# 2alaaa/distributed-llm-scheduler

Measured on AMD Instinct MI355X. Metric: DAG makespan (ms) + tasks completed under mem cap, GPT-2 DAG at 1/2/4/8 MI355X, lower is better.
Workload: dtype bf16

## Files before the change

csrc/kernels/gemm_glds_impl.h:

```cpp
#pragma once
#include <cstdlib>
#include <type_traits>
#include "common.h"
#include "kernels.h"
#include "gemm_glds_cfgs.h"

#ifndef DLS_STAMP
#define DLS_STAMP(k)
#endif

namespace {

__device__ __forceinline__ int kslice_count(int K, int kslice) { return K / kslice; }

template <int N>
__device__ __forceinline__ void wait_vm() {
  asm volatile("s_waitcnt vmcnt(%0)" ::"n"(N) : "memory");
}
template <int PW, int A>
__device__ __forceinline__ void wait_tiles(int ahead) {
  if constexpr (A == 0) {
    wait_vm<0>();
  } else {
    if (ahead >= A) wait_vm<PW * A>();
// ... 1347 lines not shown
using C31 = Cfg<192, 128, 2, 2, 2, 0, 1>;
using C32 = Cfg<192, 128, 2, 2, 3, 0, 1>;
using C33 = Cfg<192, 128, 4, 2, 3, 0, 1>;
using C34 = Cfg<256, 256, 2, 4, 2, 0, 0, 1, 1>;
using C35 = Cfg<256, 256, 2, 4, 2, 1, 0, 1, 1>;
using C36 = Cfg<256, 224, 4, 2, 2, 0, 1>;
using C37 = Cfg<256, 224, 8, 1, 2, 0, 1>;
using C38 = Cfg<128, 96, 4, 2, 4>;
using C39 = Cfg<128, 96, 2, 2, 2, 0, 0, 2>;
using C40 = Cfg<128, 64, 2, 2, 3, 0, 0, 2>;
using C41 = Cfg<192, 128, 4, 2, 3, 0, 2>;
using C42 = Cfg<256, 144, 8, 1, 3>;
using C43 = Cfg<256, 192, 4, 2, 2, 0, 1>;
using C44 = Cfg<160, 256, 2, 4, 2, 0, 1>;
using C45 = Cfg<32, 48, 2, 1, 3, 0, 0, 4>;
using C46 = Cfg<128, 128, 2, 2, 2, 0, 0, 1, 0, 2>;
using C47 = Cfg<128, 128, 2, 2, 2, 0, 1, 1, 0, 2>;

template <>
struct TallTile<C44> {
  using type = Cfg<224, 256, 2, 4, 2, 0, 1>;
};
template <>
struct TallTile<C33> {
  using type = C14;
};

template <class C>
void grouped(const GemmArgs& a, int n_groups, const int* offsets, const unsigned long long* w_ptrs,
             const unsigned long long* c_ptrs, hipStream_t s, const int* a_rows) {
  static const int w_stream = [] {
    const char* e = std::getenv("DLS_EXPERT_NT");
    return e && e[0] == '0' ? 0 : 1;
  }();
  const char* pe = std::getenv("DLS_EXPERT_PAIRS");
  const int pairs = pe && *pe ? std::atoi(pe) : 2;
  const int pair = a.grouped_shared ? 0 : pairs;
  const char* xe = std::getenv("DLS_EXPERT_XCD");
  const bool xcd = xe && *xe == '1' && !a.grouped_shared && pair != 1;
  const char* te = std::getenv("DLS_EXPERT_TALL");
  const bool tall = !(te && *te == '0') && !a.grouped_shared;
  const Epi ep{a.rope, nullptr, nullptr, nullptr, w_ptrs, c_ptrs,
               (a.grouped_shared ? 8 : ((size_t)a.M * a.lda * 2 < (1ull << 31) ? w_stream : 0)) |
                   (pair == 1 ? 16 : pair == 2 ? 32 : pair == 3 ? 64 : 0) | (xcd ? 128 : 0) | (tall ? 256 : 0)};
  const int tiles_n = (a.N + C::BN - 1) / C::BN;
  const int blocks = pair == 1 ? (n_groups * tiles_n + 7) / 8 * 16 : pair >= 2 ? 2 * n_groups * tiles_n
                                                                               : n_groups * tiles_n;
  hipLaunchKernelGGL((gemm_glds_kernel<C, 0, 3>), dim3(blocks), dim3(C::T), 0, s, (const bf16*)a.A, a.lda,
                     nullptr, a.ldw, (bf16*)a.C, a.ldc, nullptr, nullptr, 0,
                     const_cast<float*>(reinterpret_cast<const float*>(a_rows)), a.M, a.N, a.K, a.act, a.alpha,
                     n_groups, tiles_n, 1, a.K, nullptr, 0, 1e-5f, offsets, a.compact_rows, ep);
}

}

#define DLS_GLDS_DEFINE(ID)                                                                                     \
  bool glds_launch_cfg##ID(const GemmArgs& a, int splitk, float* ws, hipStream_t s, const float* ln_colsum,     \
                           int ln_mode, float ln_eps, const int* rows, bool persist) {                          \
    return launch<C##ID>(a, splitk, ws, s, ln_colsum, ln_mode, ln_eps, rows, persist);                          \
  }                                                                                                             \
  void glds_grouped_cfg##ID(const GemmArgs& a, int n_groups, const int* offsets, const unsigned long long* w_ptrs, \
                            const unsigned long long* c_ptrs, hipStream_t s, const int* a_rows) {               \
    grouped<C##ID>(a, n_groups, offsets, w_ptrs, c_ptrs, s, a_rows);                                            \
  }
```

csrc/kernels/kernels.h:

```cpp
#pragma once

#include <hip/hip_runtime_api.h>
#include <stdint.h>

constexpr int kActSwiglu = 4;

struct RopeArgs {
  const float* cos = nullptr;
  const float* sin = nullptr;
  int S = 1, D = 2, cols = 0;
};

struct GemmArgs {
  const void* A;
  int lda;
  const void* W;
  int ldw;
  void* C;
  int ldc;
  const void* bias;
  const void* R;
  int ldr;
  int M, N, K;
  int act;
  float alpha;
  int config;
  int compact_rows = 0;
  int grouped_shared = 0;
  RopeArgs rope{};
  float* stats_out = nullptr;
  const float* ext_stats = nullptr;
  int* tile_sem = nullptr;
  void* norm_out = nullptr;
  const void* norm_w = nullptr;
  const void* norm_b = nullptr;
  int norm_mode = 0;
  float norm_eps = 1e-5f;
  int ldn = 0;
  int stream_pol = 0;
};

struct Epi {
  RopeArgs rope;
  float* stats_out;
  const float* ext_stats;
  int* tile_sem = nullptr;
  const unsigned long long* grp_w = nullptr;
  const unsigned long long* grp_c = nullptr;
  int w_stream = 0;
};

int gemm_pick_config(int M, int N, int K);
void launch_gemm_bf16(const GemmArgs& a, hipStream_t s);

int gemm_glds_num_configs();
int gemm_glds_kstep(int cfg);
void gemm_glds_tile(int cfg, int* bm, int* bn);
int gemm_glds_resolve(int cfg, int act, bool ln_in);
constexpr int kGemmPersist = 64;
void gemm_glds_pick(int M, int N, int K, int* cfg, int* splitk);
size_t gemm_glds_workspace_bytes(int M, int N, int splitk);
bool launch_gemm_glds(const GemmArgs& a, int cfg, int splitk, void* workspace, hipStream_t s,
                      const float* ln_colsum = nullptr, int ln_mode = 0, float ln_eps = 1e-5f,
                      const int* rows = nullptr);
void launch_gemm_glds_grouped(const GemmArgs& a, int cfg, int n_groups, const int* offsets,
                              const unsigned long long* w_ptrs, const unsigned long long* c_ptrs, hipStream_t s,
                              const int* a_rows = nullptr);

struct GemmW8Args {
  const void* A;
  int lda;
  const void* Wq;
  int ldw;
  const float* scale;
  void* C;
  int ldc;
  const void* bias;
  const void* R;
  int ldr;
  int M, N, K;
  int act;
  float alpha;
  int config;
  int splitk;
  float* workspace;
  int store_pol;
};
int gemm_w8_num_configs();
void gemm_w8_pick(int M, int N, int K, int* cfg, int* splitk);
int gemm_w8_max_splitk(int cfg, int K);
size_t gemm_w8_workspace_bytes(int M, int N, int splitk);
void launch_gemm_w8(const GemmW8Args& a, hipStream_t s);

struct GemmW8GroupedArgs {
  const void* A;
  int lda;
  const int* a_rows;
  const int* offsets;
  const unsigned long long* w_ptrs;
  const unsigned long long* s_ptrs;
  const unsigned long long* c_ptrs;
  void* C;
  int ldc;
  int compact_rows;
  int R, N, K;
  int act;
  int n_groups;
  int config;
  int shared_weights;
  int store_pol;
};
int gemm_w8_grouped_num_configs();
int gemm_w8_grouped_tile_rows(int cfg);
int gemm_w8_grouped_pick(int rows_hint, int N, int K, int n_groups);
void launch_gemm_w8_grouped(const GemmW8GroupedArgs& a, hipStream_t s);

struct GemmW8A8Args {
// ... 269 lines not shown
```

csrc/kernels/ops_binding.cpp:

```cpp
#include <cstdlib>

#include <torch/extension.h>
#include <c10/hip/HIPStream.h>

#include "kernels.h"

namespace {

hipStream_t cur_stream() { return c10::hip::getCurrentHIPStream().stream(); }

constexpr int64_t kSemPool = 1 << 20;
int64_t sem_next[64];
int* split_k_counters(const at::Tensor& like, int64_t n) {
  static at::Tensor* pool = new at::Tensor[64];
  int64_t* next = sem_next;
  const int d = like.get_device();
  TORCH_CHECK(d >= 0 && d < 64 && n <= kSemPool, "split-K counters");
  if (!pool[d].defined()) pool[d] = at::zeros({kSemPool}, like.options().dtype(at::kInt));
  n = (n + 63) / 64 * 64;
  if (next[d] + n > kSemPool) next[d] = 0;
  int* p = pool[d].data_ptr<int>() + next[d];
  next[d] += n;
  return p;
}
int64_t split_k_cursor(int64_t device) {
  TORCH_CHECK(device >= 0 && device < 64, "split-K counters");
  return sem_next[device];
}
const bool kSplitKFixup = [] {
  const char* e = std::getenv("DLS_SPLITK_FIXUP");
  return !(e && e[0] == '0');
}();

void check_bf16(const at::Tensor& t, const char* name) {
  TORCH_CHECK(t.is_cuda(), name, " must be a GPU tensor");
  TORCH_CHECK(t.scalar_type() == at::kBFloat16, name, " must be bfloat16");
}

void check_rows(const at::Tensor& t, const char* name) {
  TORCH_CHECK(t.dim() == 2, name, " must be 2-D");
  TORCH_CHECK(t.stride(1) == 1, name, " must have contiguous rows");
  TORCH_CHECK(t.stride(0) % 8 == 0, name, " row stride must be a multiple of 8 elements");
  TORCH_CHECK(reinterpret_cast<uintptr_t>(t.data_ptr()) % 16 == 0, name, " must be 16-byte aligned");
}

at::Tensor as2d(const at::Tensor& t) { return t.dim() == 2 ? t : t.reshape({-1, t.size(-1)}); }

constexpr int64_t kRegStage = 100;

at::Tensor gemm(const at::Tensor& a_in, const at::Tensor& w, const c10::optional<at::Tensor>& bias,
                const c10::optional<at::Tensor>& residual, int64_t act, double alpha,
                const c10::optional<at::Tensor>& out, int64_t config, int64_t splitk,
                const c10::optional<at::Tensor>& ln_colsum, int64_t ln_mode, double ln_eps,
                const c10::optional<at::Tensor>& rows, bool compact_rows,
                const c10::optional<at::Tensor>& rope_cos, const c10::optional<at::Tensor>& rope_sin, int64_t rope_S,
                int64_t rope_D, int64_t rope_cols, const c10::optional<at::Tensor>& stats_out,
                const c10::optional<at::Tensor>& ext_stats, const c10::optional<at::Tensor>& norm_out,
                const c10::optional<at::Tensor>& norm_w, const c10::optional<at::Tensor>& norm_b, int64_t norm_mode,
                double norm_eps, int64_t stream_pol) {
  check_bf16(a_in, "A");
  check_bf16(w, "W");
  TORCH_CHECK(config < kRegStage + 4, "unknown GEMM config ", config, " (register-staged configs are ", kRegStage,
              "..", kRegStage + 3, ")");
  at::Tensor a = as2d(a_in);
  check_rows(a, "A");
  check_rows(w, "W");
  const int64_t M = a.size(0), K = a.size(1), N = w.size(0);
  const bool swiglu = act == kActSwiglu;
  const int64_t NO = swiglu ? N / 2 : N;
  TORCH_CHECK(w.size(1) == K, "W must be [N][K] with K = ", K, ", got ", w.sizes());
  TORCH_CHECK(K % 8 == 0, "K must be a multiple of 8");
  TORCH_CHECK(!swiglu || (N % 32 == 0 && K % 64 == 0 && !residual.has_value()),
              "SwiGLU epilogue needs N % 32 == 0, K % 64 == 0 and no residual");
  at::Tensor c;
  if (out.has_value()) {
    c = as2d(*out);
    check_bf16(c, "out");
    TORCH_CHECK((c.size(0) == M || (compact_rows && c.size(0) <= M)) && c.size(1) == NO && c.stride(1) == 1,
                "out must be [M][N_out] (or fewer rows with compact_rows)");
  } else {
    c = at::empty({M, NO}, a.options());
  }
  const void* bptr = nullptr;
  if (bias.has_value()) {
    check_bf16(*bias, "bias");
    TORCH_CHECK(bias->is_contiguous() && bias->numel() == N, "bias must be contiguous [N]");
    bptr = bias->data_ptr();
  }
  const void* rptr = nullptr;
  int ldr = 0;
  if (residual.has_value()) {
    at::Tensor r = as2d(*residual);
    check_bf16(r, "residual");
    TORCH_CHECK(r.size(0) == M && r.size(1) == N && r.stride(1) == 1, "residual must be [M][N]");
    rptr = r.data_ptr();
    ldr = (int)r.stride(0);
  }
  const int* rowp = nullptr;
  if (rows.has_value()) {
    TORCH_CHECK(rows->scalar_type() == at::kInt && rows->numel() == 2 && rows->is_contiguous() &&
                    rows->device() == a.device(),
                "rows must be a contiguous int32[2] device tensor");
    TORCH_CHECK(K % 64 == 0 && ln_mode == 0, "row-ranged GEMM needs K % 64 == 0 and no folded norm");
    rowp = rows->data_ptr<int>();
  }
  if (M == 0 || N == 0) return c;
  GemmArgs g{a.data_ptr(), (int)a.stride(0), w.data_ptr(), (int)w.stride(0), c.data_ptr(), (int)c.stride(0),
             bptr, rptr, ldr, (int)M, (int)N, (int)K, (int)act, (float)alpha, -1,
             (compact_rows && rows.has_value()) ? (int)c.size(0) : 0};
  g.stream_pol = (int)stream_pol;
  at::Tensor y_n;
  if (norm_out.has_value()) {
    TORCH_CHECK(norm_mode == 1 || norm_mode == 2, "norm_mode: 1 LayerNorm, 2 RMSNorm");
    TORCH_CHECK(!swiglu && !rows.has_value() && c.is_contiguous(), "post-norm needs a full, contiguous output");
    TORCH_CHECK(N % 8 == 0 && N <= 8192, "post-norm needs N % 8 == 0 and N <= 8192, got N = ", N);
    y_n = as2d(*norm_out);
    check_bf16(y_n, "norm_out");
    TORCH_CHECK(y_n.is_contiguous() && y_n.size(0) == M && y_n.size(1) == N, "norm_out must be contiguous [M][N]");
    TORCH_CHECK(norm_w.has_value() && norm_w->is_contiguous() && norm_w->numel() == N, "norm_w [N]");
    check_bf16(*norm_w, "norm_w");
    TORCH_CHECK(norm_mode == 2 || (norm_b.has_value() && norm_b->is_contiguous() && norm_b->numel() == N),
                "LayerNorm post-norm needs norm_b [N]");
    g.norm_out = y_n.data_ptr();
    g.ldn = (int)N;
    g.norm_w = norm_w->data_ptr();
    g.norm_b = norm_mode == 1 ? norm_b->data_ptr() : nullptr;
    g.norm_mode = (int)norm_mode;
    g.norm_eps = (float)norm_eps;
  }
  auto post_norm = [&](bool done) {
    if (!norm_out.has_value() || done) return;
    if (norm_mode == 2)
      launch_rmsnorm(c.data_ptr(), nullptr, nullptr, g.norm_w, y_n.data_ptr(), (int)M, (int)N, (float)norm_eps,
                     cur_stream());
    else
      launch_layernorm(c.data_ptr(), nullptr, nullptr, g.norm_w, g.norm_b, y_n.data_ptr(), (int)M, (int)N,
                       (float)norm_eps, cur_stream());
  };
  TORCH_CHECK(!compact_rows || (rows.has_value() && !residual.has_value()), "compact_rows needs rows and no residual");
  auto check_stats = [&](const at::Tensor& t, const char* name) {
    TORCH_CHECK(t.is_cuda() && t.scalar_type() == at::kFloat && t.is_contiguous() && t.numel() == 2 * M, name,
                " must be a contiguous fp32 [M][2] GPU tensor");
  };
  if (stats_out.has_value()) {
    check_stats(*stats_out, "stats_out");
    TORCH_CHECK(!swiglu && !rows.has_value(), "row statistics are emitted by plain (non-SwiGLU, full-row) GEMMs");
    g.stats_out = stats_out->data_ptr<float>();
  }
  if (ext_stats.has_value()) {
    check_stats(*ext_stats, "ext_stats");
    TORCH_CHECK(ln_mode != 0, "ext_stats needs ln_mode (1 LayerNorm, 2 RMSNorm) and ln_colsum");
    g.ext_stats = ext_stats->data_ptr<float>();
  }
  if (rope_cols > 0) {
    TORCH_CHECK(rope_cos.has_value() && rope_sin.has_value() && rope_cos->scalar_type() == at::kFloat &&
                    rope_sin->scalar_type() == at::kFloat && rope_cos->is_contiguous() && rope_sin->is_contiguous() &&
                    rope_cos->is_cuda() && rope_sin->is_cuda() &&
                    rope_cos->numel() >= rope_S * rope_D / 2 && rope_sin->numel() >= rope_S * rope_D / 2,
                "RoPE epilogue: cos/sin fp32 [S][D/2]");
    TORCH_CHECK(rope_D % 4 == 0 && rope_cols % rope_D == 0 && rope_cols <= N && !swiglu && K % 64 == 0 &&
                    !rows.has_value() && act == 0,
                "RoPE epilogue: D % 4 == 0, whole heads, LDS-DMA kernel, no activation / SwiGLU / row range");
    g.rope = RopeArgs{rope_cos->data_ptr<float>(), rope_sin->data_ptr<float>(), (int)rope_S, (int)rope_D,
                      (int)rope_cols};
    if (config >= kRegStage) config = -1;
  }
  const bool glds_ok = (K % 64 == 0);
  const float* csp = nullptr;
  if (ln_mode != 0) {
    TORCH_CHECK(glds_ok, "fused norm-GEMM needs K % 64 == 0");
    TORCH_CHECK(ln_colsum.has_value() && ln_colsum->scalar_type() == at::kFloat && ln_colsum->is_contiguous() &&
                    ln_colsum->numel() == N,
                "fused norm-GEMM needs fp32 ln_colsum [N]");
    csp = ln_colsum->data_ptr<float>();
  }
  if (ln_mode != 0 || swiglu || rowp || stats_out.has_value()) {
    TORCH_CHECK(glds_ok, "this epilogue needs the LDS-DMA kernel (K % 64 == 0)");
    if (config >= kRegStage) config = -1;
  }
  if (config >= kRegStage || !glds_ok) {
    g.config = config >= kRegStage ? (int)(config - kRegStage) : -1;
    launch_gemm_bf16(g, cur_stream());
    post_norm(false);
    return c;
  }
  int cfg = (int)config, sk = (int)splitk;
  if (cfg < 0 || sk <= 0) {
    int acfg, ask;
    gemm_glds_pick((int)M, (int)N, (int)K, &acfg, &ask);
    if (cfg < 0) cfg = acfg;
    if (sk <= 0) sk = ask;
  }
  TORCH_CHECK((cfg & (kGemmPersist - 1)) < gemm_glds_num_configs() && cfg < 2 * kGemmPersist, "unknown GEMM config ", cfg);
  TORCH_CHECK(K % gemm_glds_kstep(cfg) == 0, "GEMM config ", cfg, " needs K % ", gemm_glds_kstep(cfg), " == 0");
  const bool split_ok = (N % 8 == 0) && (c.stride(0) % 8 == 0) && (ldr % 8 == 0) &&
                        K % (gemm_glds_kstep(cfg) * sk) == 0 &&
                        (!swiglu || N % 32 == 0);
  if (!split_ok || (ln_mode != 0 && !ext_stats.has_value())) sk = 1;
  at::Tensor ws;
  if (sk > 1) {
    ws = at::empty({(int64_t)gemm_glds_workspace_bytes((int)M, (int)N, sk) / 4}, a.options().dtype(at::kFloat));
    if (kSplitKFixup && !rowp && !norm_out.has_value()) {
      int bm, bn;
      gemm_glds_tile(gemm_glds_resolve(cfg, (int)act, false), &bm, &bn);
      g.tile_sem = split_k_counters(a, (M + bm - 1) / bm * ((N + bn - 1) / bn));
    }
  }
  post_norm(launch_gemm_glds(g, cfg, sk, sk > 1 ? ws.data_ptr() : nullptr, cur_stream(), csp, (int)ln_mode,
                             (float)ln_eps, rowp));
  return c;
}

at::Tensor gemm_w8(const at::Tensor& a_in, const at::Tensor& wq, const at::Tensor& scale,
                   const c10::optional<at::Tensor>& bias, const c10::optional<at::Tensor>& residual, int64_t act,
                   double alpha, const c10::optional<at::Tensor>& out, int64_t config, int64_t splitk,
                   int64_t store_pol, const c10::optional<at::Tensor>& workspace) {
  check_bf16(a_in, "A");
  at::Tensor a = as2d(a_in);
  check_rows(a, "A");
  TORCH_CHECK(wq.is_cuda() && wq.device() == a.device() && wq.scalar_type() == at::kFloat8_e4m3fn,
              "W must be a float8_e4m3fn tensor on A's GPU");
  TORCH_CHECK(wq.dim() == 2, "W must be 2-D");
  const int64_t M = a.size(0), K = a.size(1), N = wq.size(0);
  TORCH_CHECK(wq.size(1) == K, "W must be [N][K] with K = ", K, ", got ", wq.sizes());
  TORCH_CHECK(K % 16 == 0, "the fp8-weight GEMM needs K % 16 == 0, got K = ", K);
  TORCH_CHECK(wq.stride(1) == 1 && wq.stride(0) % 16 == 0 && reinterpret_cast<uintptr_t>(wq.data_ptr()) % 16 == 0,
              "W must have contiguous, 16-byte aligned rows");
// ... 1281 lines not shown
}

void register_runner(py::module& m);
void register_p2p(py::module& m);

PYBIND11_MODULE(TORCH_EXTENSION_NAME, m) {
  m.doc() = "Hand-written HIP/CDNA4 (gfx950) kernels for distributed_llm_scheduler_amd";
  register_runner(m);
  register_p2p(m);
  m.def("attn_block_ok", &attn_block_ok);
  m.def("attn_block_sync_size", &attn_block_sync_size);
  m.def("attn_block", &attn_block, py::arg("x"), py::arg("w1"), py::arg("b1"), py::arg("colsum1"),
        py::arg("ext_stats"), py::arg("ln_mode"), py::arg("eps"), py::arg("qkv"), py::arg("o"), py::arg("wo"),
        py::arg("bo"), py::arg("residual"), py::arg("out"), py::arg("stats_out"), py::arg("B"), py::arg("S"),
        py::arg("n_head"), py::arg("scale"), py::arg("sync"), py::arg("spin_limit"),
        py::arg("stamps") = py::none());
  m.def("alloc_device", &alloc_device, py::arg("nbytes"), py::arg("flags") = 3);
  m.def("host_pull", &host_pull, py::arg("dst"), py::arg("src"), py::arg("blocks") = 256);
  m.def("gemm", &gemm, py::arg("a"), py::arg("w"), py::arg("bias") = py::none(), py::arg("residual") = py::none(),
        py::arg("act") = 0, py::arg("alpha") = 1.0, py::arg("out") = py::none(), py::arg("config") = -1,
        py::arg("splitk") = 0, py::arg("ln_colsum") = py::none(), py::arg("ln_mode") = 0, py::arg("ln_eps") = 1e-5,
        py::arg("rows") = py::none(), py::arg("compact_rows") = false, py::arg("rope_cos") = py::none(),
        py::arg("rope_sin") = py::none(), py::arg("rope_S") = 1, py::arg("rope_D") = 2, py::arg("rope_cols") = 0,
        py::arg("stats_out") = py::none(), py::arg("ext_stats") = py::none(), py::arg("norm_out") = py::none(),
        py::arg("norm_w") = py::none(), py::arg("norm_b") = py::none(), py::arg("norm_mode") = 0,
        py::arg("norm_eps") = 1e-5, py::arg("stream_pol") = 0);
  m.def("gemm_w8", &gemm_w8, py::arg("a"), py::arg("wq"), py::arg("scale"), py::arg("bias") = py::none(),
        py::arg("residual") = py::none(), py::arg("act") = 0, py::arg("alpha") = 1.0, py::arg("out") = py::none(),
        py::arg("config") = -1, py::arg("splitk") = 0, py::arg("store_pol") = 0, py::arg("workspace") = py::none());
  m.def("gemm_w8_num_configs", &gemm_w8_num_configs);
  m.def("gemm_w8_pick", [](int M, int N, int K) {
    int c, s;
    gemm_w8_pick(M, N, K, &c, &s);
    return std::make_pair(c, s);
  });
  m.def("gemm_grouped_w8", &gemm_grouped_w8, py::arg("x"), py::arg("weights"), py::arg("scales"), py::arg("w_ptrs"),
        py::arg("s_ptrs"), py::arg("offsets"), py::arg("act") = 0, py::arg("out") = py::none(),
        py::arg("outs") = std::vector<at::Tensor>{}, py::arg("out_ptrs") = py::none(), py::arg("config") = -1,
        py::arg("rows_hint") = 0, py::arg("a_rows") = py::none(), py::arg("shared_weights") = false,
        py::arg("store_pol") = 0);
  m.def("gemm_w8_grouped_num_configs", &gemm_w8_grouped_num_configs);
  m.def("gemm_w8_grouped_tile_rows", &gemm_w8_grouped_tile_rows);
  m.def("gemm_w8_grouped_pick", &gemm_w8_grouped_pick);
  m.def("gemm_grouped_w4a8", &gemm_grouped_w4a8, py::arg("xq"), py::arg("xscale"), py::arg("weights"),
        py::arg("scales"), py::arg("w_ptrs"), py::arg("s_ptrs"), py::arg("offsets"), py::arg("act") = 0,
        py::arg("out") = py::none(), py::arg("outs") = std::vector<at::Tensor>{}, py::arg("out_ptrs") = py::none(),
        py::arg("config") = -1, py::arg("rows_hint") = 0, py::arg("a_rows") = py::none(),
        py::arg("shared_weights") = false, py::arg("store_pol") = 0);
  m.def("gemm_w4a8_grouped_num_configs", &gemm_w4a8_grouped_num_configs);
  m.def("gemm_w4a8_grouped_tile_rows", &gemm_w4a8_grouped_tile_rows);
  m.def("gemm_w4a8_grouped_pick", &gemm_w4a8_grouped_pick);
  m.attr("REGSTAGE") = kRegStage;
  m.attr("PERSIST") = kGemmPersist;
  m.def("gemm_pick_config", &gemm_pick_config);
  m.def("gemm_glds_num_configs", &gemm_glds_num_configs);
  m.def("gemm_glds_kstep", &gemm_glds_kstep);
  m.def("gemm_glds_tile", [](int64_t cfg) {
    int bm, bn;
    gemm_glds_tile((int)cfg, &bm, &bn);
    return std::make_tuple((int64_t)bm, (int64_t)bn);
  });
  m.def("_split_k_cursor", &split_k_cursor);
  m.def("gemm_glds_pick", [](int M, int N, int K) {
    int c, s;
    gemm_glds_pick(M, N, K, &c, &s);
    return std::make_pair(c, s);
  });
  m.def("attention", &attention, py::arg("q"), py::arg("k"), py::arg("v"), py::arg("B"), py::arg("S"),
        py::arg("n_head"), py::arg("n_kv_head"), py::arg("head_dim"), py::arg("causal") = true,
        py::arg("scale") = 0.125, py::arg("out") = py::none(), py::arg("variant") = 0, py::arg("Sq") = 0,
        py::arg("q_off") = 0, py::arg("flags") = 0);
  m.def("kv_append", &kv_append, py::arg("k_new"), py::arg("v_new"), py::arg("k_cache"), py::arg("v_cache"),
        py::arg("pos"), py::arg("T"), py::arg("k_scale") = py::none(), py::arg("v_scale") = py::none());
  m.def("attention_decode_sizes", &attention_decode_sizes, py::arg("B"), py::arg("T"), py::arg("C"),
        py::arg("n_head"), py::arg("n_kv_head"), py::arg("head_dim"), py::arg("chunk") = 0);
  m.def("attention_decode_chunk", [](int64_t B, int64_t C, int64_t n_kv_head, int64_t head_dim) {
    return (int64_t)attn_decode_chunk((int)B, (int)C, (int)n_kv_head, (int)head_dim);
  });
  m.def("attention_decode", &attention_decode, py::arg("q"), py::arg("k_cache"), py::arg("v_cache"), py::arg("pos"),
        py::arg("T"), py::arg("n_head"), py::arg("n_kv_head"), py::arg("head_dim"), py::arg("scale"),
        py::arg("part"), py::arg("cnt"), py::arg("out") = py::none(), py::arg("chunk") = 0,
        py::arg("k_scale") = py::none(), py::arg("v_scale") = py::none());
  m.def("decode_prologue", &decode_prologue, py::arg("pos"), py::arg("tokens"), py::arg("tok_out"), py::arg("T"),
        py::arg("C"), py::arg("tables"), py::arg("outs"));
  m.def("sample_sizes", &sample_sizes_b, py::arg("B"), py::arg("V"));
  m.def("sample_tokens", &sample_tokens, py::arg("logits"), py::arg("V"), py::arg("T"), py::arg("pos"),
        py::arg("tokens"), py::arg("C"), py::arg("temperature"), py::arg("top_k"), py::arg("top_p"), py::arg("seed"),
        py::arg("request"), py::arg("prompt_len"), py::arg("eos"), py::arg("done"), py::arg("next_out"),
        py::arg("stats"), py::arg("part"), py::arg("cnt"));
  m.def("norm", &norm, py::arg("x"), py::arg("w"), py::arg("b") = py::none(), py::arg("eps") = 1e-5,
        py::arg("residual") = py::none(), py::arg("rms") = false, py::arg("out") = py::none(),
        py::arg("sum_out") = py::none());
  m.def("gemm_w8a8", &gemm_w8a8, py::arg("xq"), py::arg("xscale"), py::arg("wq"), py::arg("scale"),
        py::arg("bias") = py::none(), py::arg("residual") = py::none(), py::arg("act") = 0, py::arg("alpha") = 1.0,
        py::arg("out") = py::none(), py::arg("config") = -1, py::arg("splitk") = 0, py::arg("store_pol") = 0,
        py::arg("workspace") = py::none());
  m.def("gemm_w8a8_num_configs", &gemm_w8a8_num_configs);
  m.def("gemm_w8a8_pick", [](int M, int N, int K) {
    int c, s;
    gemm_w8a8_pick(M, N, K, &c, &s);
    return std::make_pair(c, s);
  });
  m.def("gemm_w4a8", &gemm_w4a8, py::arg("xq"), py::arg("xscale"), py::arg("wq"), py::arg("ws"),
        py::arg("bias") = py::none(), py::arg("residual") = py::none(), py::arg("act") = 0, py::arg("alpha") = 1.0,
        py::arg("out") = py::none(), py::arg("config") = -1, py::arg("splitk") = 0, py::arg("store_pol") = 0,
        py::arg("workspace") = py::none());
// ... 39 lines not shown
```

distributed_llm_scheduler_amd/ops/__init__.py:

```python
from __future__ import annotations

import math
import os
import threading
from typing import Optional, Tuple

import torch
import torch.nn.functional as F

from . import tuning

ACT = {None: 0, "none": 0, "gelu": 1, "gelu_tanh": 1, "silu": 2, "relu": 3, "swiglu": 4}
SWIGLU = 4
SWIGLU_BLOCK = 16
LMHEAD_POL = int(os.environ.get("DLS_LMHEAD_POL", "3"))
LMHEAD_MIN_N = 32000
WEIGHT_NT_MB = float(os.environ.get("DLS_WEIGHT_NT_MB", "0"))
ACT_POL = int(os.environ.get("DLS_ACT_POL", "4"))
ACT_POL_MODEL = {"mixtral-8x7b": 0}
_ACT_POL_SET = "DLS_ACT_POL" in os.environ
ATTN_FLAGS = int(os.environ.get("DLS_ATTN_FLAGS", "0"))
ATTN_VARIANT = int(os.environ.get("DLS_ATTN_VARIANT", "0"))


# ... 147 lines not shown
def ref_rope_(qkv, S, n_head, n_kv_head, head_dim, k_col, cos_t, sin_t):
    M = qkv.shape[0]
    pos = torch.arange(M, device=qkv.device) % S
    c, s = cos_t[pos].to(qkv.device), sin_t[pos].to(qkv.device)
    half = head_dim // 2

    def rot(view, heads):
        x = view.float().reshape(M, heads, head_dim)
        x1, x2 = x[..., :half], x[..., half:]
        cc, ss = c[:, None, :], s[:, None, :]
        out = torch.cat([x1 * cc - x2 * ss, x2 * cc + x1 * ss], dim=-1)
        view.copy_(out.reshape(M, heads * head_dim).to(view.dtype))

    rot(qkv[:, :n_head * head_dim], n_head)
    rot(qkv[:, k_col:k_col + n_kv_head * head_dim], n_kv_head)
    return qkv



def _post_norm_args(post_norm):
    y, nw, nb, kind, eps = post_norm
    return dict(norm_out=y, norm_w=nw, norm_b=nb if kind == "layernorm" else None,
                norm_mode=1 if kind == "layernorm" else 2, norm_eps=float(eps))


def _post_norm_ref(src, post_norm):
    y, nw, nb, kind, eps = post_norm
    s2 = src.reshape(-1, src.shape[-1])
    r = ref_layernorm(s2, nw, nb, eps) if kind == "layernorm" else ref_rmsnorm(s2, nw, eps)
    y.view(r.shape).copy_(r)


def linear(x, w, bias=None, act=None, residual=None, alpha=1.0, out=None, rows=None, rows_hint=None,
           compact=False, rope=None, stats_out=None, post_norm=None):
    a = ACT[act] if not isinstance(act, int) else act
    n_out = w.shape[0] // 2 if a == SWIGLU else w.shape[0]
    if _gpu(x):
        shp = x.shape[:-1] + (n_out,)
        M = x.numel() // x.shape[-1]
        cfg, sk = tuning.lookup(rows_hint or M, w.shape[0], w.shape[1], tuning.tag(a, rows is not None))
        if cfg == tuning.LIB:
            if tuning.VENDOR and a == 0 and residual is None and rows is None and rope is None \
                    and stats_out is None and post_norm is None:
                x2 = x.reshape(M, x.shape[-1])
                o2 = out.view(M, n_out) if out is not None else torch.empty(M, n_out, dtype=x.dtype, device=x.device)
                if bias is not None:
                    torch.addmm(bias, x2, w.t(), beta=1.0, alpha=float(alpha), out=o2)
                else:
                    torch.mm(x2, w.t(), out=o2)
                    if alpha != 1.0:
                        o2.mul_(alpha)
                return o2.view(shp) if out is None else out
            cfg, sk = tuning.lookup_fused(rows_hint or M, w.shape[0], w.shape[1], tuning.tag(a, rows is not None))
        rc, rs_, rS, rD, rcols = rope if rope is not None else (None, None, 1, 2, 0)
        y = ext().gemm(x, w, bias, residual, a, float(alpha), out, cfg, sk, None, 0, 1e-5, rows, bool(compact),
                       rc, rs_, int(rS), int(rD), int(rcols), stats_out, None,
                       stream_pol=_stream_pol(w.shape[0], w.shape[1]) if rows is None else 0,
                       **(_post_norm_args(post_norm) if post_norm is not None else {}))
        return y.view(shp) if out is None else out
    if rows is not None:
        r0, r1 = (int(v) for v in rows.tolist())
        if out is None:
            out = torch.zeros(x.shape[:-1] + (n_out,), dtype=x.dtype)
        res = residual[r0:r1] if residual is not None else None
        o2 = out.reshape(-1, out.shape[-1])
        if compact:
            n = min(r1 - r0, o2.shape[0])
            o2[:n] = ref_linear(x[r0:r0 + n], w, bias, act, None, alpha)
        else:
            o2[r0:r1] = ref_linear(x[r0:r1], w, bias, act, res, alpha)
        return out
    y = ref_linear(x, w, bias, act, residual, alpha, rope=rope)
    if out is not None:
        out.copy_(y)
        y = out
    if post_norm is not None:
        _post_norm_ref(y, post_norm)
    return y


def quantize_fp8(w):
    from ..models.params import quantize_fp8 as _q
    return _q(w)


def dequantize_fp8(q, scale, dtype=torch.bfloat16):
    from ..models.params import dequantize_fp8 as _d
    return _d(q, scale, dtype)


W8_SPLITS = (1, 2, 4, 8)


def w8_configs() -> int:
    return int(ext().gemm_w8_num_configs())


def w8_workspace_elems(M: int, N: int, K: int) -> int:
    _, sk = ext().gemm_w8_pick(int(M), int(N), int(K))
    return int(sk) * int(M) * int(N) if sk > 1 else 0


def linear_w8(x, q, scale, bias=None, act=None, residual=None, alpha=1.0, out=None, config=None, workspace=None):
    a = ACT[act] if not isinstance(act, int) else act
    if q.dtype != torch.float8_e4m3fn:
        raise TypeError(f"linear_w8: the weight must be float8_e4m3fn, got {q.dtype}")
# ... 117 lines not shown
        raise TypeError(f"linear_w4a8: the activations must be float8_e4m3fn, got {xq.dtype}")
    if q.dtype != torch.uint8 or s.dtype != torch.uint8:
        raise TypeError(f"linear_w4a8: the MXFP4 weight and its block scales must be uint8, got {q.dtype} and {s.dtype}")
    K = xq.shape[-1]
    if K % 32:
        raise ValueError(f"linear_w4a8: K must be a multiple of 32, got {K}")
    if q.dim() != 2 or q.shape[1] != K // 2 or tuple(s.shape) != (q.shape[0], K // 32):
        raise ValueError(f"linear_w4a8: expected q [N, {K // 2}] and s [N, {K // 32}], got {tuple(q.shape)} and "
                         f"{tuple(s.shape)}")
    if _gpu(xq):
        n_out = q.shape[0] // 2 if a == SWIGLU else q.shape[0]
        cfg, sk = (-1, 0) if config is None else (tuple(config) if isinstance(config, (tuple, list)) else (config, 1))
        y = ext().gemm_w4a8(xq, xscale, q, s, bias, residual, a, float(alpha), out, int(cfg), int(sk),
                            _stream_pol(q.shape[0], K) & 6, workspace)
        return y.view(xq.shape[:-1] + (n_out,)) if out is None else out
    xd = dequantize_fp8(xq.reshape(-1, K), xscale, torch.float32).reshape(xq.shape)
    y = ref_linear(xd, dequantize_mxfp4(q, s, torch.float32), bias, act, residual, alpha).to(torch.bfloat16)
    if out is not None:
        out.copy_(y.reshape(out.shape))
        return out
    return y


def derive_norm_gemm(w, ln_w, ln_b=None, bias=None):
    wf = w.float()
    wd = (wf * ln_w.float()[None, :]).to(w.dtype)
    cs = wd.float().sum(1).contiguous()
    b = torch.zeros(w.shape[0], device=w.device) if bias is None else bias.float()
    if ln_b is not None:
        b = b + (wf * ln_b.float()[None, :]).sum(1)
    return wd, cs, b.to(w.dtype).contiguous()


def linear_norm(x, w_derived, colsum, bias_derived, mode, eps=1e-5, act=None, residual=None, out=None, rope=None,
                ext_stats=None):
    m = {"layernorm": 1, "rmsnorm": 2}[mode]
    a = ACT[act] if not isinstance(act, int) else act
    shp = x.shape[:-1] + (w_derived.shape[0] // 2 if a == SWIGLU else w_derived.shape[0],)
    M, N, K = x.numel() // x.shape[-1], w_derived.shape[0], w_derived.shape[1]
    split = tuning.col_split(M, N, K, tuning.tag(a)) if ext_stats is not None and rope is None and a != SWIGLU \
        else None
    if split:
        if out is None:
            out = torch.empty(shp, dtype=x.dtype, device=x.device)
        o2 = out.view(M, N)
        r2 = residual.reshape(M, N) if residual is not None else None
        pol = _stream_pol(N, K)
        for n0, n1, c, k in split:
            ext().gemm(x, w_derived[n0:n1], bias_derived[n0:n1] if bias_derived is not None else None,
                       r2[:, n0:n1] if r2 is not None else None, a, 1.0, o2[:, n0:n1], int(c), int(k),
                       colsum[n0:n1], m, float(eps), None, False, None, None, 1, 2, 0, None, ext_stats,
                       stream_pol=pol)
        return out
    cfg, sk = tuning.lookup_fused(M, N, K, tuning.tag(a))
    if ext_stats is None:
        sk = 1
        if 0 <= cfg < tuning.REGSTAGE and tuning.kstep(cfg) != 64:
            cfg = next((int(c) for c, _ in tuning.runner_ups(M, N, K, tuning.tag(a), 8)
                        if 0 <= c < tuning.REGSTAGE and tuning.kstep(c) == 64), -1)
    rc, rs_, rS, rD, rcols = rope if rope is not None else (None, None, 1, 2, 0)
    pol = _stream_pol(N, K)
    y = ext().gemm(x, w_derived, bias_derived, residual, a, 1.0, out, cfg if cfg < tuning.REGSTAGE else -1, sk, colsum,
                   m, float(eps), None, False, rc, rs_, int(rS), int(rD), int(rcols), None, ext_stats,
                   stream_pol=pol)
    return y.view(shp) if out is None else out


def mlp_fused_ok(M, H, F, Hout) -> bool:
    return bool(ext().mlp_fused_ok(int(M), int(H), int(F), int(Hout)))


def mlp_fused(x, w1_derived, b1_derived, colsum1, ext_stats, mode, eps, h, w2, b2, residual, out, stats_out=None,
              sync=None, spin_limit=1 << 22):
    m = {"layernorm": 1, "rmsnorm": 2}[mode]
    if sync is None:
        sync = torch.zeros(2 * (x.numel() // x.shape[-1]) // 64 + 1, dtype=torch.int32, device=x.device)
    ext().mlp_fused(x, w1_derived, b1_derived, colsum1, ext_stats, m, float(eps), ACT["gelu"], h, w2, b2, residual,
                    out, stats_out, sync, int(spin_limit))
    return out


def attn_block_ok(M, H, B, S, n_head, n_kv_head, head_dim) -> bool:
    return bool(ext().attn_block_ok(int(M), int(H), int(B), int(S), int(n_head), int(n_kv_head), int(head_dim)))


def attn_block_sync(M, S, B, n_head, device) -> torch.Tensor:
    return torch.zeros(int(ext().attn_block_sync_size(int(M), int(S), int(B), int(n_head))), dtype=torch.int32,
                       device=device)


def attn_block(x, w_qkv_derived, b_qkv_derived, colsum, ext_stats, mode, eps, qkv, o, w_o, b_o, residual, out,
               B, S, n_head, stats_out=None, sync=None, scale=None, spin_limit=1 << 22):
    m = {"layernorm": 1, "rmsnorm": 2}[mode]
    H = x.shape[-1]
    if sync is None:
        sync = attn_block_sync(x.numel() // H, S, B, n_head, x.device)
    scale = scale if scale is not None else 1.0 / math.sqrt(H // n_head)
    ext().attn_block(x, w_qkv_derived, b_qkv_derived, colsum, ext_stats, m, float(eps), qkv, o, w_o, b_o, residual,
                     out, stats_out, int(B), int(S), int(n_head), float(scale), sync, int(spin_limit))
    return out


def layernorm(x, w, b, eps=1e-5, residual=None, out=None, sum_out=None):
    if _gpu(x):
        y, s = ext().norm(x, w, b, float(eps), residual, False, out, sum_out)
        y = y.view(x.shape)
        return (y, s.view(x.shape)) if residual is not None else y
# ... 620 lines not shown
```

distributed_llm_scheduler_amd/ops/tuning.py:

```python
from __future__ import annotations

import json
import os
import statistics
import threading
from typing import Dict, Iterable, Optional, Tuple

import torch

_PATH = os.environ.get("DLS_GEMM_TUNING") or os.path.join(os.path.dirname(os.path.abspath(__file__)),
                                                          "gemm_tuning.json")
_lock = threading.Lock()
_table: Optional[Dict[str, Tuple[int, int]]] = None
_cands: Dict[str, list] = {}
_refined: Dict[str, bool] = {}
_col_splits: Dict[str, list] = {}
_overrides: Dict[str, Dict[str, Tuple[int, int]]] = {}
_model: Optional[str] = None
REGSTAGE = 100
PERSIST = 64
LIB = 200
VENDOR = os.environ.get("DLS_ALLOW_VENDOR_GEMM", "0") == "1"


def _key(M: int, N: int, K: int, tg: str = "") -> str:
    return f"{M}x{N}x{K}{tg}"


def tag(act: int = 0, ranged: bool = False) -> str:
    return ("s" if act == 4 else "") + ("r" if ranged else "")


def table() -> Dict[str, Tuple[int, int]]:
    global _table
    with _lock:
        if _table is None:
            _table = {}
            if os.path.exists(_PATH):
                try:
                    with open(_PATH) as f:
                        doc = json.load(f)
                    _table = {k: tuple(v) for k, v in doc.get("gemm", {}).items()}
                    _cands.update({k: [tuple(c) for c in v] for k, v in doc.get("candidates", {}).items()})
                    _refined.update(doc.get("refined", {}))
                    _col_splits.update({k: [tuple(x) for x in v] for k, v in doc.get("col_splits", {}).items()})
                    _overrides.update({m: {k: tuple(v) for k, v in t.items()}
                                       for m, t in doc.get("model_overrides", {}).items()})
                except (OSError, ValueError):
                    _table = {}
        return _table


def set_model(name: Optional[str]) -> None:
    global _model
    _model = name


def lookup(M: int, N: int, K: int, tg: str = "") -> Tuple[int, int]:
    t = table()
    v = _overrides.get(_model, {}).get(_key(M, N, K, tg))
    if v is not None:
        return v
    v = t.get(_key(M, N, K, tg))
    if v is None and tg:
        v = t.get(_key(M, N, K))
        if v is not None and v[0] >= REGSTAGE:
            v = None
    if v is not None and v[0] == LIB and not VENDOR:
        v = _hip_candidate(M, N, K, tg)
    return v if v is not None else (-1, 0)


def _hip_candidate(M: int, N: int, K: int, tg: str = ""):
    for c in _cands.get(_key(M, N, K, tg), []):
        if c[0] != LIB:
# ... 198 lines not shown
```

Before: 0.5501.

## Add wave-private LDS ring GEMM kernel with in-block split-K reduction

```diff
diff --git a/csrc/kernels/gemm_glds_impl.h b/csrc/kernels/gemm_glds_impl.h
--- a/csrc/kernels/gemm_glds_impl.h
+++ b/csrc/kernels/gemm_glds_impl.h
@@ -1423,6 +1423,240 @@
                      n_groups, tiles_n, 1, a.K, nullptr, 0, 1e-5f, offsets, a.compact_rows, ep);
 }
 
+template <int W_, int S_>
+struct PrivCfg {
+  static constexpr int W = W_, S = S_, BM = 32, BN = 48, BK = 64, CH = 8, FM = 2, FN = 3;
+  static constexpr int T = 64 * W, PW = (BM + BN) / 8;
+  static constexpr int SLOT = (BM + BN) * CH;
+  static constexpr int RING = S * SLOT, LDS_UNITS = W * RING;
+  static constexpr int REG = FM * FN * 64;
+  static_assert(S >= 1 && PW * (S - 1) <= 63, "vmcnt range");
+  static_assert(LDS_UNITS * 16 <= 163840 && T <= 1024, "LDS budget, block size");
+  static_assert(REG <= RING, "a wave's fragment region lies inside its own ring");
+  static_assert(T >= BM * 8, "one 16-byte output segment per storing thread");
+};
+
+template <class P>
+__device__ __forceinline__ void mainloop_private(bf16x8* ring, const bf16* __restrict__ A, int lda,
+                                                 const bf16* __restrict__ W, int ldw, int M, int N, int m0, int n0,
+                                                 int kbeg, int nk, int lane, f32x4 (&acc)[P::FM][P::FN]) {
+  const bf16* src[P::PW];
+#pragma unroll
+  for (int j = 0; j < P::PW; ++j) {
+    const int row = 8 * j + (lane >> 3);
+    const int kofs = kbeg + ((lane & 7) ^ (row & 7)) * 8;
+    src[j] = row < P::BM ? A + (size_t)min(m0 + row, M - 1) * lda + kofs
+                         : W + (size_t)min(n0 + row - P::BM, N - 1) * ldw + kofs;
+  }
+  auto issue = [&](int kt, bf16x8* slot) {
+#pragma unroll
+    for (int j = 0; j < P::PW; ++j)
+      __builtin_amdgcn_global_load_lds((const void*)(src[j] + kt * P::BK),
+                                       (__attribute__((address_space(3))) void*)(slot + j * 64), 16, 0, 0);
+  };
+#pragma unroll
+  for (int s = 0; s < P::S; ++s)
+    if (s < nk) issue(s, ring + s * P::SLOT);
+  int sl = 0;
+  for (int kt = 0; kt < nk; ++kt) {
+    wait_tiles<P::PW, P::S - 1>(min(P::S - 1, nk - 1 - kt));
+    bf16x8* slot = ring + sl * P::SLOT;
+    const bf16x8* sA = slot;
+    const bf16x8* sB = slot + P::BM * P::CH;
+    bf16x8 af[2][P::FM], bw[2][P::FN];
+#pragma unroll
+    for (int kk = 0; kk < 2; ++kk) {
+      const int chunk = kk * 4 + (lane >> 4);
+#pragma unroll
+      for (int j = 0; j < P::FN; ++j) {
+        const int row = j * 16 + (lane & 15);
+        bw[kk][j] = sB[row * P::CH + (chunk ^ (row & 7))];
+      }
+#pragma unroll
+      for (int i = 0; i < P::FM; ++i) {
+        const int row = i * 16 + (lane & 15);
+        af[kk][i] = sA[row * P::CH + (chunk ^ (row & 7))];
+      }
+    }
+    __builtin_amdgcn_sched_barrier(0);
+    asm volatile("s_waitcnt lgkmcnt(0)" ::: "memory");
+    __builtin_amdgcn_sched_barrier(0);
+    if (kt + P::S < nk) issue(kt + P::S, slot);
+    __builtin_amdgcn_sched_barrier(0);
+#pragma unroll
+    for (int kk = 0; kk < 2; ++kk)
+#pragma unroll
+      for (int i = 0; i < P::FM; ++i)
+#pragma unroll
+        for (int j = 0; j < P::FN; ++j) acc[i][j] = mfma16x16x32(bw[kk][j], af[kk][i], acc[i][j]);
+    sl = sl + 1 == P::S ? 0 : sl + 1;
+  }
+}
+
+template <class P, int SPOL>
+__global__ __launch_bounds__(P::T, 1) void gemm_private_kernel(const bf16* __restrict__ A, int lda,
+                                                               const bf16* __restrict__ W, int ldw,
+                                                               bf16* __restrict__ Cp, int ldc,
+                                                               const bf16* __restrict__ bias,
+                                                               const bf16* __restrict__ R, int ldr,
+                                                               float* __restrict__ stats_out, int M, int N, int K,
+                                                               float alpha, int tiles_m) {
+  __shared__ bf16x8 smem[P::LDS_UNITS];
+  const int tid = threadIdx.x, lane = tid & 63;
+  const int wave = __builtin_amdgcn_readfirstlane(tid >> 6);
+  const int tile = xcd_remap(blockIdx.x, gridDim.x);
+  const int m0 = (tile % tiles_m) * P::BM, n0 = (tile / tiles_m) * P::BN;
+  DLS_STAMP(0)
+  const int nk = K / (P::BK * P::W);
+  bf16x8* ring = smem + wave * P::RING;
+  f32x4 acc[P::FM][P::FN];
+#pragma unroll
+  for (int i = 0; i < P::FM; ++i)
+#pragma unroll
+    for (int j = 0; j < P::FN; ++j) acc[i][j] = f32x4{0.f, 0.f, 0.f, 0.f};
+  mainloop_private<P>(ring, A, lda, W, ldw, M, N, m0, n0, wave * nk * P::BK, nk, lane, acc);
+  DLS_STAMP(1)
+  constexpr int BNC = P::BN / 8, BNP = 8;
+  const bool own = tid < P::BM * BNP;
+  const int rl = tid / BNP, cc = tid % BNP;
+  const int row = m0 + rl, col = n0 + cc * 8;
+  const bool pre_bvec = ((reinterpret_cast<uintptr_t>(bias) & 7) | (N & 3)) == 0;
+  const bool v16 = ((reinterpret_cast<uintptr_t>(Cp) | ((uintptr_t)ldc * 2)) & 15) == 0 &&
+                   (!R || ((reinterpret_cast<uintptr_t>(R) | ((uintptr_t)ldr * 2)) & 15) == 0);
+  const bool pre_res = R != nullptr && N >= 8 && v16 && ((size_t)(M + P::BM) * ldr * 2 < (1ull << 31));
+  u32x2 o_bv[2];
+  u32x4 o_r;
+  if (own) {
+    constexpr int kRaw = 0x00020000;
+    if (bias && pre_bvec) {
+      const auto rs = __builtin_amdgcn_make_buffer_rsrc(const_cast<bf16*>(bias), 0, N * 2, kRaw);
+#pragma unroll
+      for (int h = 0; h < 2; ++h) o_bv[h] = __builtin_amdgcn_raw_buffer_load_b64(rs, col * 2 + h * 8, 0, 0);
+    }
+    if (pre_res) {
+      const auto rs =
+          __builtin_amdgcn_make_buffer_rsrc(const_cast<bf16*>(R), 0, (int)(((size_t)(M - 1) * ldr + N) * 2), kRaw);
+      o_r = __builtin_amdgcn_raw_buffer_load_b128(rs, (row * ldr + col) * 2, 0, 0);
+    }
+  }
+  f32x4* reg = reinterpret_cast<f32x4*>(ring);
+#pragma unroll
+  for (int i = 0; i < P::FM; ++i)
+#pragma unroll
+    for (int j = 0; j < P::FN; ++j) {
+      const int cl = j * 16 + (lane >> 4) * 4;
+      reg[(i * P::FN + j) * 64 + (lane & 48) + ((lane & 15) ^ (((cl >> 3) & 3) << 2))] = acc[i][j];
+    }
+  epi_barrier<true>();
+  DLS_STAMP(7)
+  if (own) {
+    const int ccr = min(cc, BNC - 1), cl0 = ccr * 8;
+    const int rec = ((rl / 16) * P::FN + cl0 / 16) * 64 + (cl0 & 8) * 4 + ((rl & 15) ^ ((ccr & 3) << 2));
+    const f32x4* red = reinterpret_cast<const f32x4*>(smem);
+    f32x4 part_lo[P::W], part_hi[P::W];
+#pragma unroll
+    for (int w = 0; w < P::W; ++w) {
+      part_lo[w] = red[w * P::RING + rec];
+      part_hi[w] = red[w * P::RING + rec + 16];
+    }
+    f32x4 lo = part_lo[0], hi = part_hi[0];
+#pragma unroll
+    for (int w = 1; w < P::W; ++w) {
+      lo += part_lo[w];
+      hi += part_hi[w];
+    }
+    float bv[8] = {0.f, 0.f, 0.f, 0.f, 0.f, 0.f, 0.f, 0.f};
+    if (bias) {
+      if (pre_bvec) {
+        uint32_t w[8];
+#pragma unroll
+        for (int h = 0; h < 2; ++h) {
+          consume_from_here(o_bv[h]);
+          const uint32_t p0 = o_bv[h][0], p1 = o_bv[h][1];
+          w[4 * h + 0] = p0 << 16;
+          w[4 * h + 1] = p0 & 0xffff0000u;
+          w[4 * h + 2] = p1 << 16;
+          w[4 * h + 3] = p1 & 0xffff0000u;
+        }
+#pragma unroll
+        for (int e = 0; e < 8; ++e) bv[e] = col + e < N ? __uint_as_float(w[e]) : 0.f;
+      } else {
+#pragma unroll
+        for (int e = 0; e < 8; ++e)
+          if (col + e < N) bv[e] = bf2f(bias[col + e]);
+      }
+    }
+    bf16x8 o;
+#pragma unroll
+    for (int e = 0; e < 8; ++e) o[e] = f2bf(alpha * (e < 4 ? lo[e & 3] : hi[e & 3]) + bv[e]);
+    if (pre_res) consume_from_here(o_r);
+    float s1 = 0.f, s2 = 0.f;
+    if (cc < BNC && row < M && col < N) {
+      if (v16 && col + 8 <= N) {
+        if (R) {
+          const bf16x8 r8 = pre_res ? *reinterpret_cast<const bf16x8*>(&o_r)
+                                    : *reinterpret_cast<const bf16x8*>(R + (size_t)row * ldr + col);
+#pragma unroll
+          for (int e = 0; e < 8; ++e) o[e] = f2bf(bf2f(o[e]) + bf2f(r8[e]));
+        }
+        store16_pol<SPOL>(Cp, ((size_t)row * ldc + col) * 2, *reinterpret_cast<const u32x4*>(&o));
+#pragma unroll
+        for (int e = 0; e < 8; ++e) {
+          const float y = bf2f(o[e]);
+          s1 += y;
+          s2 += y * y;
+        }
+      } else {
+#pragma unroll
+        for (int e = 0; e < 8; ++e) {
+          if (col + e >= N) continue;
+          float x = bf2f(o[e]);
+          if (R) x += bf2f(R[(size_t)row * ldr + col + e]);
+          const bf16 ob = f2bf(x);
+          Cp[(size_t)row * ldc + col + e] = ob;
+          const float y = bf2f(ob);
+          s1 += y;
+          s2 += y * y;
+        }
+      }
+    }
+    if (stats_out) {
+#pragma unroll
+      for (int o_ = 1; o_ < BNP; o_ <<= 1) {
+        s1 += __shfl_xor(s1, o_, 64);
+        s2 += __shfl_xor(s2, o_, 64);
+      }
+      if (cc == 0 && row < M) {
+        atomicAdd(stats_out + 2 * row, s1);
+        atomicAdd(stats_out + 2 * row + 1, s2);
+      }
+    }
+  }
+  DLS_STAMP(3)
+}
+
+inline bool private_takes(int waves, const GemmArgs& a, int splitk, bool folded_norm, bool ranged) {
+  return waves > 0 && a.K > 0 && a.K % (64 * waves) == 0 && splitk <= 1 && !folded_norm && !ranged &&
+         a.act == ACT_NONE && a.rope.cols == 0 && !a.ext_stats;
+}
+
+template <int W_, int S_>
+void launch_private(const GemmArgs& a, hipStream_t s) {
+  using P = PrivCfg<W_, S_>;
+  const int tiles_m = (a.M + P::BM - 1) / P::BM, tiles_n = (a.N + P::BN - 1) / P::BN;
+  dim3 grid(tiles_m * tiles_n), block(P::T);
+#define DLS_PK(POL_)                                                                                               \
+  hipLaunchKernelGGL((gemm_private_kernel<P, POL_>), grid, block, 0, s, (const bf16*)a.A, a.lda, (const bf16*)a.W, \
+                     a.ldw, (bf16*)a.C, a.ldc, (const bf16*)a.bias, (const bf16*)a.R, a.ldr, a.stats_out, a.M, a.N, \
+                     a.K, a.alpha, tiles_m)
+  switch ((size_t)a.M * a.ldc * 2 < (1ull << 31) ? a.stream_pol & 7 : 0) {
+    case 2: case 3: DLS_PK(kPolStream); break;
+    case 4: case 5: DLS_PK(kPolWT); break;
+    default: DLS_PK(0);
+  }
+#undef DLS_PK
+}
+
 }
 
 #define DLS_GLDS_DEFINE(ID)                                                                                     \
diff --git a/csrc/kernels/gemm_private.hip b/csrc/kernels/gemm_private.hip
--- /dev/null
+++ b/csrc/kernels/gemm_private.hip
@@ -0,0 +1,24 @@
+#include "gemm_glds_impl.h"
+
+namespace {
+constexpr int kWaves[kGemmPrivateCount] = {8, 4, 6, 12};
+}
+
+int gemm_private_waves(int cfg) {
+  return cfg >= kGemmPrivate && cfg < kGemmPrivate + kGemmPrivateCount ? kWaves[cfg - kGemmPrivate] : 0;
+}
+
+bool gemm_private_takes(const GemmArgs& a, int cfg, int splitk, bool folded_norm, bool ranged) {
+  return private_takes(gemm_private_waves(cfg), a, splitk, folded_norm, ranged);
+}
+
+bool launch_gemm_private(const GemmArgs& a, int cfg, hipStream_t s) {
+  if (!gemm_private_takes(a, cfg, 1, false, false)) return false;
+  switch (cfg - kGemmPrivate) {
+    case 0: launch_private<8, 2>(a, s); break;
+    case 1: launch_private<4, 3>(a, s); break;
+    case 2: launch_private<6, 2>(a, s); break;
+    default: launch_private<12, 1>(a, s); break;
+  }
+  return true;
+}
diff --git a/csrc/kernels/kernels.h b/csrc/kernels/kernels.h
--- a/csrc/kernels/kernels.h
+++ b/csrc/kernels/kernels.h
@@ -63,6 +63,11 @@
 bool launch_gemm_glds(const GemmArgs& a, int cfg, int splitk, void* workspace, hipStream_t s,
                       const float* ln_colsum = nullptr, int ln_mode = 0, float ln_eps = 1e-5f,
                       const int* rows = nullptr);
+constexpr int kGemmPrivate = 120, kGemmPrivateCount = 4;
+int gemm_private_waves(int cfg);
+bool gemm_private_takes(const GemmArgs& a, int cfg, int splitk, bool folded_norm, bool ranged);
+bool launch_gemm_private(const GemmArgs& a, int cfg, hipStream_t s);
+
 void launch_gemm_glds_grouped(const GemmArgs& a, int cfg, int n_groups, const int* offsets,
                               const unsigned long long* w_ptrs, const unsigned long long* c_ptrs, hipStream_t s,
                               const int* a_rows = nullptr);
diff --git a/csrc/kernels/ops_binding.cpp b/csrc/kernels/ops_binding.cpp
--- a/csrc/kernels/ops_binding.cpp
+++ b/csrc/kernels/ops_binding.cpp
@@ -60,8 +60,10 @@
                 double norm_eps, int64_t stream_pol) {
   check_bf16(a_in, "A");
   check_bf16(w, "W");
-  TORCH_CHECK(config < kRegStage + 4, "unknown GEMM config ", config, " (register-staged configs are ", kRegStage,
-              "..", kRegStage + 3, ")");
+  const bool priv = gemm_private_waves((int)config) != 0;
+  TORCH_CHECK(config < kRegStage + 4 || priv, "unknown GEMM config ", config, " (register-staged configs are ",
+              kRegStage, "..", kRegStage + 3, ", wave-private rings ", kGemmPrivate, "..",
+              kGemmPrivate + kGemmPrivateCount - 1, ")");
   at::Tensor a = as2d(a_in);
   check_rows(a, "A");
   check_rows(w, "W");
@@ -163,7 +165,7 @@
                 "RoPE epilogue: D % 4 == 0, whole heads, LDS-DMA kernel, no activation / SwiGLU / row range");
     g.rope = RopeArgs{rope_cos->data_ptr<float>(), rope_sin->data_ptr<float>(), (int)rope_S, (int)rope_D,
                       (int)rope_cols};
-    if (config >= kRegStage) config = -1;
+    if (config >= kRegStage && !priv) config = -1;
   }
   const bool glds_ok = (K % 64 == 0);
   const float* csp = nullptr;
@@ -173,6 +175,15 @@
                     ln_colsum->numel() == N,
                 "fused norm-GEMM needs fp32 ln_colsum [N]");
     csp = ln_colsum->data_ptr<float>();
+  }
+  if (priv) {
+    TORCH_CHECK(!compact_rows && gemm_private_takes(g, (int)config, (int)splitk, ln_mode != 0, rowp != nullptr),
+                "GEMM config ", config, " (wave-private rings, ", gemm_private_waves((int)config),
+                " waves) takes plain launches only: K % ", 64 * gemm_private_waves((int)config),
+                " == 0, no activation, folded norm, RoPE, SwiGLU, split-K or row range");
+    TORCH_CHECK(launch_gemm_private(g, (int)config, cur_stream()), "GEMM config ", config, " refused the launch");
+    post_norm(false);
+    return c;
   }
   if (ln_mode != 0 || swiglu || rowp || stats_out.has_value()) {
     TORCH_CHECK(glds_ok, "this epilogue needs the LDS-DMA kernel (K % 64 == 0)");
@@ -1560,6 +1571,9 @@
   m.def("gemm_w4a8_grouped_pick", &gemm_w4a8_grouped_pick);
   m.attr("REGSTAGE") = kRegStage;
   m.attr("PERSIST") = kGemmPersist;
+  m.attr("PRIVATE") = kGemmPrivate;
+  m.attr("PRIVATE_COUNT") = kGemmPrivateCount;
+  m.def("gemm_private_waves", &gemm_private_waves);
   m.def("gemm_pick_config", &gemm_pick_config);
   m.def("gemm_glds_num_configs", &gemm_glds_num_configs);
   m.def("gemm_glds_kstep", &gemm_glds_kstep);
diff --git a/distributed_llm_scheduler_amd/ops/__init__.py b/distributed_llm_scheduler_amd/ops/__init__.py
--- a/distributed_llm_scheduler_amd/ops/__init__.py
+++ b/distributed_llm_scheduler_amd/ops/__init__.py
@@ -223,6 +223,7 @@
                         o2.mul_(alpha)
                 return o2.view(shp) if out is None else out
             cfg, sk = tuning.lookup_fused(rows_hint or M, w.shape[0], w.shape[1], tuning.tag(a, rows is not None))
+        cfg, sk = tuning.resolve_private((cfg, sk), w.shape[1], a, rows is not None, rope is not None)
         rc, rs_, rS, rD, rcols = rope if rope is not None else (None, None, 1, 2, 0)
         y = ext().gemm(x, w, bias, residual, a, float(alpha), out, cfg, sk, None, 0, 1e-5, rows, bool(compact),
                        rc, rs_, int(rS), int(rD), int(rcols), stats_out, None,
@@ -446,7 +447,7 @@
                        colsum[n0:n1], m, float(eps), None, False, None, None, 1, 2, 0, None, ext_stats,
                        stream_pol=pol)
         return out
-    cfg, sk = tuning.lookup_fused(M, N, K, tuning.tag(a))
+    cfg, sk = tuning.resolve_private(tuning.lookup_fused(M, N, K, tuning.tag(a)), K, a, folded=True)
     if ext_stats is None:
         sk = 1
         if 0 <= cfg < tuning.REGSTAGE and tuning.kstep(cfg) != 64:
diff --git a/distributed_llm_scheduler_amd/ops/tuning.py b/distributed_llm_scheduler_amd/ops/tuning.py
--- a/distributed_llm_scheduler_amd/ops/tuning.py
+++ b/distributed_llm_scheduler_amd/ops/tuning.py
@@ -21,6 +21,23 @@
 PERSIST = 64
 LIB = 200
 VENDOR = os.environ.get("DLS_ALLOW_VENDOR_GEMM", "0") == "1"
+PRIVATE = 120
+PRIVATE_WAVES = {120: 8, 121: 4, 122: 6, 123: 12}
+PRIVATE_FALLBACK = (45, 1)
+
+
+def private_takes(cfg: int, K: int, sk: int = 1, act: int = 0, ranged: bool = False, rope: bool = False,
+                  folded: bool = False) -> bool:
+    w = PRIVATE_WAVES.get(cfg, 0)
+    return w > 0 and K > 0 and K % (64 * w) == 0 and sk <= 1 and act == 0 and not (ranged or rope or folded)
+
+
+def resolve_private(choice: Tuple[int, int], K: int, act: int = 0, ranged: bool = False, rope: bool = False,
+                    folded: bool = False) -> Tuple[int, int]:
+    cfg, sk = choice
+    if cfg not in PRIVATE_WAVES:
+        return choice
+    return (cfg, 1) if private_takes(cfg, K, sk, act, ranged, rope, folded) else PRIVATE_FALLBACK
 
 
 def _key(M: int, N: int, K: int, tg: str = "") -> str:
```

After: 0.5345, median of 6. 2.8% less time.
